# lhoyer/improving_segmentation_with_selfsupervised_depth

Measured on AMD Instinct MI355X. Metric: train images/sec, ResNet-101 joint seg+depth @512x1024, higher is better.
Workload: dtype f32

## Files before the change

### improving_segmentation_with_selfsupervised_depth_amd/csrc/conv_igemm.hip

```cpp
#include <type_traits>
#include "segsde_common.h"
#include "conv_small.h"
#include "winograd.h"
#include <cstdlib>
#include <mutex>
#include <cstring>

namespace {

struct ConvP {
  const float* x0; const float* x1; const float* w; const float* bias;
  float* y; float* y2;
  int B, H, W, C0, C1, ld0, ld1, up0;
  int Ho, Wo, N, ldy, ldy2, nsplit;
  int KH, KW, stride, dil, pad, pad_mode, in_div;
  int Ctot, Ktot, M, act, sum2x2;
  int vecout;
  int nb, ne;
  const float* zero;
  int kh0, khs, kw0, kws, KWf, Kfull, os, oph, opw, OHf, OWf;
  double* stats;
  int accum;
  const float* agy; int agld, agkind;
  unsigned mg1, mg2; int sf1, sf2, d1, d2;
  unsigned mgC, mgKW; int sfC, sfKW;
  int lin;
  int padw, wtap, osfast;
  int submap;
  int tapskip;
  long wbstride;
  int cmp;
};
constexpr int SEGSDE_PAD_CLAMP_ = 3;

struct KInfo {
  const float* src; int ld, Hs, Ws, shift, dh, dw, cc; bool valid;
};

__device__ __forceinline__ int fast_div(int n, unsigned magic, int shift) {
  return magic ? (int)(__umulhi((unsigned)n, magic) >> shift) : n;
}

__device__ __forceinline__ KInfo decode_k(const ConvP& p, int k) {
  KInfo t;
  t.valid = k < p.Ktot;
  const int kk = t.valid ? k : 0;
  const int tap = fast_div(kk, p.mgC, p.sfC), c = kk - tap * p.Ctot;
  const int kh = fast_div(tap, p.mgKW, p.sfKW), kw = tap - kh * p.KW;
  t.dh = kh * p.dil - p.pad;
  t.dw = kw * p.dil - p.pad;
  if (c < p.C0) { t.src = p.x0; t.ld = p.ld0; t.cc = c; t.shift = p.up0; }
  else { t.src = p.x1; t.ld = p.ld1; t.cc = c - p.C0; t.shift = 0; }
  t.Hs = p.H >> t.shift;
  t.Ws = p.W >> t.shift;
  return t;
}
// ... 678 lines not shown
      if (sn < pe.ne) {
        double* pr = pe.stats + ((long)(mt * R + sl) * 2) * pe.N + sn;
        pr[0] = ((s8[0] + s8[1]) + (s8[2] + s8[3])) + ((s8[4] + s8[5]) + (s8[6] + s8[7]));
        pr[pe.N] = ((q8[0] + q8[1]) + (q8[2] + q8[3])) + ((q8[4] + q8[5]) + (q8[6] + q8[7]));
      }
    }
    constexpr int CQ = BN / 4, RPP = 256 / CQ;
    const int cq = tid % CQ, rr = tid / CQ;
    const int n = n0 + 4 * cq;
    {
      const int nend = n0 + BN < pe.ne ? n0 + BN : pe.ne;
      const bool side1 = n0 >= pe.nsplit;
      if ((!pe.submap || pe.osfast) && m0 + BM <= pe.M && (side1 || nend <= pe.nsplit)) {
        constexpr int NR = BM / RPP;
        const long row0 = pe.submap ? out_row(pe, m0) : (long)m0;
        float* dbase = side1 ? pe.y2 + (row0 * pe.ldy2 + (n0 - pe.nsplit)) : pe.y + (row0 * pe.ldy + n0);
        const unsigned ld = (unsigned)(side1 ? pe.ldy2 : pe.ldy) * (unsigned)pe.os;
        const segsde_rsrc rd = segsde_make_rsrc(dbase);
        const unsigned vo = n < pe.ne ? ((unsigned)rr * ld + 4u * cq) * 4u : SEGSDE_OOB;
        const unsigned step = (unsigned)RPP * ld * 4u;
        const bool ag = pe.agy && !side1;
        const unsigned agl = (unsigned)pe.agld * (unsigned)pe.os;
        const segsde_rsrc ra = segsde_make_rsrc(ag ? pe.agy + (row0 * pe.agld + n0) : pe.zero);
        const unsigned voa = (ag && n < pe.ne) ? ((unsigned)rr * agl + 4u * cq) * 4u : SEGSDE_OOB;
        const unsigned stepa = (unsigned)RPP * agl * 4u;
        const float* cp = Ct + rr * BN + 4 * cq;
        float4 o[NR];
        if (pe.accum) {
          unsigned so = 0;
#pragma unroll
          for (int t = 0; t < NR; ++t) { o[t] = segsde_buffer_load4(rd, vo, so); so += step; }
        }
        unsigned so = 0, soa = 0;
        if (pe.accum && pe.act != SEGSDE_ACT_NONE) {
#pragma unroll
          for (int t = 0; t < NR; ++t) {
            float4 v = *reinterpret_cast<const float4*>(cp + t * RPP * BN);
            v.x += o[t].x; v.y += o[t].y; v.z += o[t].z; v.w += o[t].w;
            if (pe.act == SEGSDE_ACT_ELU) {
              v.x = v.x > 0.f ? v.x : __expf(fminf(v.x, 0.f)) - 1.f; v.y = v.y > 0.f ? v.y : __expf(fminf(v.y, 0.f)) - 1.f;
              v.z = v.z > 0.f ? v.z : __expf(fminf(v.z, 0.f)) - 1.f; v.w = v.w > 0.f ? v.w : __expf(fminf(v.w, 0.f)) - 1.f;
            } else {
              v.x = segsde_act(v.x, pe.act); v.y = segsde_act(v.y, pe.act); v.z = segsde_act(v.z, pe.act); v.w = segsde_act(v.w, pe.act);
            }
            segsde_buffer_store4(rd, vo, so, v);
            so += step;
          }
          return;
        }
#pragma unroll
        for (int t = 0; t < NR; ++t) {
          float4 v = *reinterpret_cast<const float4*>(cp + t * RPP * BN);
          if (ag) {
            const float4 yv = segsde_buffer_load4(ra, voa, soa);
            v.x *= segsde_act_grad_from_out(yv.x, pe.agkind); v.y *= segsde_act_grad_from_out(yv.y, pe.agkind);
            v.z *= segsde_act_grad_from_out(yv.z, pe.agkind); v.w *= segsde_act_grad_from_out(yv.w, pe.agkind);
          }
          if (pe.accum) { v.x += o[t].x; v.y += o[t].y; v.z += o[t].z; v.w += o[t].w; }
          segsde_buffer_store4(rd, vo, so, v);
          so += step; soa += stepa;
        }
        return;
      }
    }
    if (n < pe.ne) {
      float* dst; long ld; int nn;
      if (n < pe.nsplit) { dst = pe.y; ld = pe.ldy; nn = n; }
      else { dst = pe.y2; ld = pe.ldy2; nn = n - pe.nsplit; }
      if (pe.accum) {
        constexpr int NR = BM / RPP;
        float4 o[NR];
        const float* ag = (pe.agy && n < pe.nsplit) ? pe.agy + nn : nullptr;
#pragma unroll
        for (int t = 0; t < NR; ++t) {
          const int m = m0 + rr + t * RPP;
          o[t] = make_float4(0.f, 0.f, 0.f, 0.f);
          if (m < pe.M) o[t] = *reinterpret_cast<const float4*>(dst + out_row(pe, m) * ld + nn);
        }
#pragma unroll
        for (int t = 0; t < NR; ++t) {
          const int ml = rr + t * RPP, m = m0 + ml;
          if (m < pe.M) {
            float4 v = *reinterpret_cast<const float4*>(Ct + ml * BN + 4 * cq);
            if (ag) {
              const float4 yv = *reinterpret_cast<const float4*>(ag + out_row(pe, m) * pe.agld);
              v.x *= segsde_act_grad_from_out(yv.x, pe.agkind); v.y *= segsde_act_grad_from_out(yv.y, pe.agkind);
              v.z *= segsde_act_grad_from_out(yv.z, pe.agkind); v.w *= segsde_act_grad_from_out(yv.w, pe.agkind);
            }
            v.x += o[t].x; v.y += o[t].y; v.z += o[t].z; v.w += o[t].w;
            if (pe.act == SEGSDE_ACT_ELU) {
              v.x = v.x > 0.f ? v.x : __expf(fminf(v.x, 0.f)) - 1.f; v.y = v.y > 0.f ? v.y : __expf(fminf(v.y, 0.f)) - 1.f;
              v.z = v.z > 0.f ? v.z : __expf(fminf(v.z, 0.f)) - 1.f; v.w = v.w > 0.f ? v.w : __expf(fminf(v.w, 0.f)) - 1.f;
            } else if (pe.act != SEGSDE_ACT_NONE) {
              v.x = segsde_act(v.x, pe.act); v.y = segsde_act(v.y, pe.act); v.z = segsde_act(v.z, pe.act); v.w = segsde_act(v.w, pe.act);
            }
            *reinterpret_cast<float4*>(dst + out_row(pe, m) * ld + nn) = v;
          }
        }
      } else if (pe.agy && n < pe.nsplit) {
        const float* ag = pe.agy + nn;
#pragma unroll 4
        for (int ml = rr; ml < BM; ml += RPP) {
          const int m = m0 + ml;
          if (m < pe.M) {
            const long row = out_row(pe, m);
            float4 v = *reinterpret_cast<const float4*>(Ct + ml * BN + 4 * cq);
            const float4 yv = *reinterpret_cast<const float4*>(ag + row * pe.agld);
            v.x *= segsde_act_grad_from_out(yv.x, pe.agkind); v.y *= segsde_act_grad_from_out(yv.y, pe.agkind);
            v.z *= segsde_act_grad_from_out(yv.z, pe.agkind); v.w *= segsde_act_grad_from_out(yv.w, pe.agkind);
            *reinterpret_cast<float4*>(dst + row * ld + nn) = v;
          }
        }
      } else {
#pragma unroll 4
        for (int ml = rr; ml < BM; ml += RPP) {
          const int m = m0 + ml;
          if (m < pe.M) {
            float4* q = reinterpret_cast<float4*>(dst + out_row(pe, m) * ld + nn);
            *q = *reinterpret_cast<const float4*>(Ct + ml * BN + 4 * cq);
          }
        }
      }
// ... 634 lines not shown
  const unsigned long long num = 1ULL << (31 + l);
  magic = (unsigned)((num + (unsigned long long)d - 1) / (unsigned long long)d);
  shift = l - 1;
}
void set_divs(ConvP& p) {
  p.d1 = p.sum2x2 ? (p.Ho >> 1) * (p.Wo >> 1) : p.Ho * p.Wo;
  p.d2 = p.sum2x2 ? (p.Wo >> 1) : p.Wo;
  magic_for(p.d1, p.mg1, p.sf1);
  magic_for(p.d2, p.mg2, p.sf2);
  magic_for(p.Ctot, p.mgC, p.sfC);
  magic_for(p.KW, p.mgKW, p.sfKW);
}

ConvP make_params(const segsde_conv_desc* d, const float* x0, const float* x1, const float* w, const float* bias,
                  float* y, float* y2) {
  ConvP p;
  p.x0 = x0; p.x1 = x1 ? x1 : x0; p.w = w; p.bias = bias; p.y = y; p.y2 = y2 ? y2 : y;
  p.B = d->B; p.H = d->H; p.W = d->W; p.C0 = d->C0; p.C1 = d->C1; p.ld0 = d->ld0; p.ld1 = d->C1 ? d->ld1 : d->ld0;
  p.up0 = d->up0; p.Ho = d->Ho; p.Wo = d->Wo; p.N = d->Cout; p.ldy = d->ldy;
  p.ldy2 = d->ldy2 ? d->ldy2 : d->ldy; p.nsplit = y2 ? d->nsplit : d->Cout;
  p.KH = d->KH; p.KW = d->KW; p.stride = d->stride; p.dil = d->dil; p.pad = d->pad; p.pad_mode = d->pad_mode;
  p.in_div = d->in_div < 1 ? 1 : d->in_div;
  p.Ctot = d->C0 + d->C1; p.Ktot = d->KH * d->KW * p.Ctot; p.M = d->B * d->Ho * d->Wo; p.act = d->act;
  p.sum2x2 = d->sum2x2;
  set_divs(p);
  p.nb = 0; p.ne = p.N;
  p.vecout = (p.N % 4 == 0) && (p.ldy % 4 == 0) && (p.ldy2 % 4 == 0) && (p.nsplit % 4 == 0) && aligned16(p.y) &&
             aligned16(p.y2);
  p.zero = zero_page();
  p.kh0 = 0; p.khs = 1; p.kw0 = 0; p.kws = 1; p.KWf = p.KW; p.Kfull = p.Ktot; p.os = 1; p.oph = 0; p.opw = 0; p.OHf = p.Ho; p.OWf = p.Wo;
  p.stats = nullptr;
  p.accum = d->accumulate ? 1 : 0;
  p.cmp = (d->compute == 1 || d->compute == 2) ? d->compute : 0;
  p.agy = nullptr; p.agld = 0; p.agkind = 0;
  p.lin = d->KH == 1 && d->KW == 1 && d->stride == 1 && d->pad == 0 && d->in_div <= 1 && !d->up0 && !d->sum2x2 && d->C1 == 0 &&
          d->H == d->Ho && d->W == d->Wo;
  p.padw = p.pad; p.wtap = p.Ctot; p.osfast = 0; p.submap = 0;
  p.tapskip = (d->pad_mode == SEGSDE_PAD_ZERO && d->dil > 1 && d->KH > 1 && d->in_div <= 1 && !d->up0 && !d->sum2x2 &&
               d->stride == 1) ? 1 : 0;
  p.wbstride = 0;
  return p;
}


bool vec_ok(const ConvP& p) {
  return (p.Ctot % 4 == 0) && (p.C0 % 4 == 0) && (p.ld0 % 4 == 0) && (p.ld1 % 4 == 0) && aligned16(p.x0) &&
         aligned16(p.x1) && aligned16(p.w);
}

int validate(const segsde_conv_desc* d) {
  if (!d || d->B <= 0 || d->H <= 0 || d->W <= 0 || d->C0 <= 0 || d->C1 < 0 || d->Cout <= 0) return SEGSDE_ERR_SHAPE;
  if (d->KH <= 0 || d->KW <= 0 || d->stride <= 0 || d->dil <= 0 || d->pad < 0) return SEGSDE_ERR_SHAPE;
  if (d->up0 && ((d->H & 1) || (d->W & 1))) return SEGSDE_ERR_SHAPE;
  if (d->pad_mode == SEGSDE_PAD_REFLECT && (d->pad >= d->H || d->pad >= d->W)) return SEGSDE_ERR_SHAPE;
  if (d->pad_mode == SEGSDE_PAD_REFLECT_ADJOINT &&
      (d->KH != 3 || d->KW != 3 || d->stride != 1 || d->dil != 1 || d->pad != 1 || d->in_div > 1 || d->C1 != 0 ||
       d->H != d->Ho || d->W != d->Wo || d->H < 2 || d->W < 2))
    return SEGSDE_ERR_SHAPE;
  if (d->ld0 < d->C0 || (d->C1 && d->ld1 < d->C1) || d->ldy <= 0) return SEGSDE_ERR_SHAPE;
  if (d->compute == 3) return SEGSDE_ERR_UNSUPPORTED;
  return 0;
}

bool fast_ok(const ConvP& p) {
  const long e0 = (long)p.B * (p.H >> p.up0) * (p.W >> p.up0) * p.ld0;
  const long e1 = (long)p.B * p.H * p.W * p.ld1;
  return vec_ok(p) && (p.Ctot % 32 == 0) && (p.C1 == 0 || p.C0 % 32 == 0) && p.in_div <= 2 && e0 < (1L << 31) &&
// ... 175 lines not shown
}

extern "C" int segsde_reflect_adjoint_borders(const segsde_conv_desc* d, const float* dy, const float* wdpack, float* y,
                                              const float* act_out, int act_ld, int act_kind, void* stream) {
  if (!dy || !wdpack || !y) return SEGSDE_ERR_NULL;
  ConvP p;
  if (int e = borders_params(d, dy, wdpack, y, act_out, act_ld, act_kind, p)) return e;
  return launch_adjoint_by_borders(p, static_cast<hipStream_t>(stream), false);
}

extern "C" long segsde_conv2d_stats_rows(const segsde_conv_desc* d) {
  if (validate(d)) return 0;
  float dummy[4];
  const ConvP p = make_params(d, dummy, dummy, dummy, nullptr, reinterpret_cast<float*>(16), nullptr);
  return stats_rows(d, p);
}

extern "C" int segsde_conv2d_forward(const segsde_conv_desc* d, const float* x0, const float* x1, const float* wpack,
                                     const float* bias, float* y, float* y2, void* stream) {
  return segsde_conv2d_forward_stats(d, x0, x1, wpack, bias, y, y2, nullptr, stream);
}

extern "C" int segsde_conv2d_forward_stats(const segsde_conv_desc* d, const float* x0, const float* x1, const float* wpack,
                                           const float* bias, float* y, float* y2, double* stats, void* stream) {
  return segsde_conv2d_dgrad_actgrad(d, x0, x1, wpack, bias, y, y2, stats, nullptr, 0, 0, stream);
}

extern "C" int segsde_conv2d_dgrad_actgrad(const segsde_conv_desc* d, const float* x0, const float* x1, const float* wpack,
                                           const float* bias, float* y, float* y2, double* stats, const float* act_out,
                                           int act_ld, int act_kind, void* stream) {
  if (int e = validate(d)) return e;
  if (!x0 || !wpack || !y || (d->C1 && !x1)) return SEGSDE_ERR_NULL;
  ConvP p = make_params(d, x0, x1, wpack, bias, y, y2);
  if (act_out) {
    if (stats || bias || d->act != 0 || act_kind < SEGSDE_ACT_RELU || act_kind > SEGSDE_ACT_SIGMOID || act_ld < p.nsplit ||
        (act_ld % 4) || !aligned16(act_out) || d->in_div > 1)
      return SEGSDE_ERR_UNSUPPORTED;
    p.agy = act_out; p.agld = act_ld; p.agkind = act_kind;
  }
  if (stats) {
    if (stats_rows(d, p) == 0) return SEGSDE_ERR_UNSUPPORTED;
    p.stats = stats;
  }
  const bool parity_split = d->in_div == 2 && d->stride == 1 && (d->dil & 1) && d->pad_mode == SEGSDE_PAD_ZERO && !d->sum2x2 &&
                            d->C1 == 0 && !d->up0 && !bias && d->act == 0 && !y2 && p.vecout;
  if (d->accumulate) {
    if (y2 || bias || d->act != 0 || d->sum2x2 || (d->in_div > 1 && !parity_split) || !p.vecout || d->Cout == 1 || d->C0 % 4 != 0 ||
        d->C0 == 1 || (d->pad_mode == SEGSDE_PAD_REFLECT_ADJOINT && !igemm_fast_ok(p)))
      return SEGSDE_ERR_UNSUPPORTED;
  }
  hipStream_t s = static_cast<hipStream_t>(stream);
  const bool plain3x3 = d->KH == 3 && d->KW == 3 && d->stride == 1 && d->dil == 1 && d->pad == 1 && d->C1 == 0 && !d->up0 &&
                        d->in_div <= 1 && !d->sum2x2 && d->H == d->Ho && d->W == d->Wo;
  if (plain3x3 && d->Cout == 1 && d->pad_mode != SEGSDE_PAD_REFLECT_ADJOINT && segsde_c1_supported(d->C0, d->ld0) &&
      aligned16(x0) && aligned16(wpack))
    return probing() ? 0 : segsde_c1_forward(x0, d->ld0, d->B, d->H, d->W, d->C0, wpack, bias, d->pad_mode == SEGSDE_PAD_REFLECT, d->act, y,
                             d->ldy, stream);
  if (plain3x3 && d->C0 == 1 && d->pad_mode != SEGSDE_PAD_REFLECT && !bias && d->act == 0 &&
      segsde_c1_supported(d->Cout, p.ldy) && p.vecout)
    return probing() ? 0 : segsde_c1_dgrad(x0, d->ld0, d->B, d->H, d->W, d->Cout, wpack, d->pad_mode == SEGSDE_PAD_REFLECT_ADJOINT, y, p.ldy,
                           y2, p.ldy2, p.nsplit, p.agy, p.agld, p.agkind, stream);
  const bool plain1x1 = d->KH == 1 && d->KW == 1 && d->stride == 1 && d->pad == 0 && d->C1 == 0 && !d->up0 && d->in_div <= 1 &&
                        !d->sum2x2 && d->H == d->Ho && d->W == d->Wo;
  if (plain1x1 && !stats && !p.agy && d->C0 % 4 != 0 && d->ld0 == d->C0 && aligned16(x0) && !bias && d->act == 0 && !y2 &&
      segsde_skinny_supported(d->C0, d->Cout) && p.vecout)
    return probing() ? 0 : segsde_skinny_nk(x0, d->C0, wpack, (long)d->B * d->H * d->W, d->Cout, y, p.ldy, stream);
  if (parity_split) {
    bool ok = true;
    ConvP sub[4]; int nsub = 0; bool empty = false;
    for (int ph = 0; ph < 2 && ok; ++ph)
      for (int pw = 0; pw < 2 && ok; ++pw) {
// ... 836 lines not shown
```

### improving_segmentation_with_selfsupervised_depth_amd/functional.py

```python
import collections
import weakref

import torch
from torch.autograd import Function as _TorchFunction

from . import hipops as H


class Function(_TorchFunction):

    @classmethod
    def apply(cls, *args):
        return super(_TorchFunction, cls).apply(*args)


FUSIONS = {}


def _grad_dest(param):
    from . import ddp
    return ddp.grad_destination(param) if ddp._GRAD_DEST else None


def fp32_region(fn):
# ... 95 lines not shown

def to_nchw_dense(x_nhwc):
    return _ToNCHWDense.apply(x_nhwc)


class StemFn(Function):

    @staticmethod
    def forward(ctx, image, weight, mean, std, stats_out=None, wstem=None):
        xpad = H.stem_input(image, mean, std)
        if wstem is None:
            wstem = H.stem_pack(weight)
        C = weight.shape[1]
        if stats_out is not None:
            y, part = H.stem_forward(xpad, wstem, C, want_stats=True)
            stats_out.append(part)
        else:
            y = H.stem_forward(xpad, wstem, C)
        ctx.C = C
        ctx.save_for_backward(xpad)
        return y

    @staticmethod
    def backward(ctx, dy):
        (xpad,) = ctx.saved_tensors
        dw = H.stem_wgrad(xpad, _c(dy), ctx.C) if ctx.needs_input_grad[1] else None
        return None, dw, None, None, None, None


class ConvFn(Function):

    @staticmethod
    def forward(ctx, x0, x1, weight, bias, g, act, stats_out=None, grad_box=None, packs=None, x0_act=None, act_box=None,
                fold_cache=None, wino_cache=None, skip_box=None):
        ctx.grad_box = grad_box
        ctx.skip_box = skip_box
        ctx.x0_act, ctx.act_box = x0_act, act_box
        x0 = _c(x0) if x0.stride(-1) != 1 else x0
        ctx.wd = None
        ctx.wd_gen = None
        if packs is not None:
            wp, ctx.wd = packs
            ctx.wd_gen = getattr(ctx.wd, "_segsde_gen", None)
        elif ctx.needs_input_grad[0] or (x1 is not None and ctx.needs_input_grad[1]):
            wp, ctx.wd = H.pack_weight_both(weight)
        else:
            wp = H.pack_weight(weight, False)
        ctx.wp = wp if g.reflect else None
        ctx.fold = None
        ctx.wino = None
        up_f = 2 if g.up0 else 1
        kn = H.winograd_fused_ok(g, x0.shape[0], x0.shape[1] * up_f, x0.shape[2] * up_f)
        kn_d2 = (x1 is not None and g.up0 and (ctx.needs_input_grad[1])
                 and H.winograd_fused_dgrad2_ok(g, x0.shape[0], x0.shape[1] * up_f, x0.shape[2] * up_f))
        if kn or kn_d2 or (not g.up0 and H.winograd_ok(g, x0.shape[0], x0.shape[1], x0.shape[2])):
            knl = kn or kn_d2
            if (wino_cache is not None and wino_cache.get("key") is not None and wino_cache.get("key") == wino_cache.get("want")
                    and bool(wino_cache.get("kn")) == knl):
                ctx.wino = wino_cache["packs"]
            else:
                ctx.wino = H.winograd_pack(weight, kn=knl)
                if wino_cache is not None and wino_cache.get("want") is not None:
                    wino_cache["packs"], wino_cache["key"], wino_cache["kn"] = ctx.wino, wino_cache["want"], knl
        wino_f = None if (ctx.wino is None or (kn_d2 and not kn)) else ctx.wino[0]
        keep_v = wino_f is not None and not kn and ctx.needs_input_grad[2]
        H.WINO_V[0] = None
        if stats_out is not None:
            y, part = H.conv_forward(g, x0, x1, wp, bias, act, want_stats=True, wino=wino_f, keep_v=keep_v)
# ... 6 lines not shown
                    ctx.fold = H.upfold_pack(weight, g.C0)
                    if fold_cache is not None and fold_cache.get("want") is not None:
                        fold_cache["fold"], fold_cache["key"] = ctx.fold, fold_cache["want"]
            y = H.conv_forward(g, x0, x1, wp, bias, act, wfold=None if ctx.fold is None else ctx.fold[0], wino=wino_f, keep_v=keep_v)
        ctx.wino_v, H.WINO_V[0] = H.WINO_V[0], None
        ctx.g, ctx.act = g, act
        ctx.in_hw = (x0.shape[1] * (2 if g.up0 else 1), x0.shape[2] * (2 if g.up0 else 1))
        ctx.has_bias = bias is not None
        ctx.save_for_backward(x0, x1, weight)
        return y

    @staticmethod
    def backward(ctx, dy):
        x0, x1, weight = ctx.saved_tensors
        g = ctx.g
        dz = _c(dy)
        need_b = ctx.has_bias and ctx.needs_input_grad[3]
        dbias = None
        if need_b:
            stash = ctx.act_box.pop("dbias", None) if ctx.act_box is not None else None
            same = stash is not None and stash[0].data_ptr() == dz.data_ptr() and stash[0]._version == stash[1] == dz._version
            dbias = stash[2] if same else H.colsum(dz)
            fusion("bias_grad_from_activation_pass", bool(same))
        actgrad = (x0, ctx.x0_act) if ctx.x0_act is not None else None
        dx0 = dx1 = dw = None
        if ctx.needs_input_grad[0] or (x1 is not None and ctx.needs_input_grad[1]):
            wd = ctx.wd if ctx.wd is not None else H.pack_weight(weight, True)
            if ctx.wd_gen is not None and getattr(wd, "_segsde_gen", None) != ctx.wd_gen:
                raise RuntimeError("the weight packs of this graph were rebuilt by a later weight_pack_scope(model): a graph "
                                   "must be consumed before the next prepack of the same weights")
            dx0 = None
            box = ctx.grad_box
            if box is not None and box.get("g") is not None and x1 is None:
                dx0, dx1 = H.conv_dgrad(g, dz, wd, weight.detach(), ctx.in_hw, accumulate_into=box["g"], actgrad=actgrad,
                                        wino=None if ctx.wino is None else ctx.wino[1], wfpack=ctx.wp)
                if dx0 is not None:
                    box["fused"] = True
            if dx0 is None:
                sbox = ctx.skip_box if (x1 is not None and ctx.needs_input_grad[1]) else None
                dx0, dx1 = H.conv_dgrad(g, dz, wd, weight.detach(), ctx.in_hw, actgrad=actgrad, fold=ctx.fold,
                                        need0=ctx.needs_input_grad[0], need1=x1 is not None and ctx.needs_input_grad[1],
                                        wino=None if ctx.wino is None else ctx.wino[1],
                                        accumulate_skip_into=None if sbox is None else sbox.get("g"), wfpack=ctx.wp)
                if sbox is not None and dx1 is not None:
                    if H.SKIP_ACCUMULATED[0]:
                        sbox["fused"] = True
                    elif sbox.get("publish") and sbox.get("g") is None and dx1.is_contiguous():
                        sbox["g"] = dx1
                        sbox["fused"] = True
                if box is not None and box.get("publish") and box.get("g") is None and x1 is None and not g.up0 \
                        and dx0.is_contiguous():
                    box["g"] = dx0
                    box["fused"] = True
            if actgrad is not None and ctx.needs_input_grad[0]:
                fusion("activation_backward_in_dgrad_epilogue", bool(H.ACTGRAD_FUSED[0]))
            if not ctx.needs_input_grad[0]:
                dx0 = None
            if x1 is None or not ctx.needs_input_grad[1]:
                dx1 = None
        if ctx.needs_input_grad[2]:
            dw = H.conv_wgrad(g, x0, x1, dz, wino_v=ctx.wino_v, out=_grad_dest(weight))
            ctx.wino_v = None
        return dx0, dx1, dw, dbias, None, None, None, None, None, None, None, None, None, None


class ActGradFn(Function):

    passes = 0

    @staticmethod
    def forward(ctx, y, act, box):
        ctx.act, ctx.box = act, box
        ctx.save_for_backward(y)
        return y.view_as(y)

    @staticmethod
    def backward(ctx, dy):
        (y,) = ctx.saved_tensors
        ActGradFn.passes += 1
        fusion("activation_backward_in_dgrad_epilogue", False)
        dz, dbias = H.act_backward(_c(dy), y, ctx.act, need_dbias=bool(ctx.box.get("need_dbias")))
        if dbias is not None:
            ctx.box["dbias"] = (dz, dz._version, dbias)
        return dz, None, None


class BNActFn(Function):

    @staticmethod
    def forward(ctx, x, gamma, beta, residual, running_mean, running_var, training, momentum, eps, act, drop_p, seed,
                partials=None, grad_box=None, nbt=None):
        ctx.grad_box = grad_box
        x = _c(x)
        if training and partials is not None:
            mean, invstd = H.bn_stats_from_partials(partials, x.numel() // x.shape[-1], running_mean, running_var, momentum,
                                                    eps, update_running=running_mean is not None, num_batches_tracked=nbt)
        elif training:
            mean, invstd = H.bn_stats(x, running_mean, running_var, momentum, eps, update_running=running_mean is not None,
                                      num_batches_tracked=nbt)
        else:
            mean, invstd = H.bn_eval_stats(running_mean, running_var, eps)
        y = H.bn_apply(x, mean, invstd, gamma, beta, residual, act, drop_p, seed)
        remask = act in ("none", "relu") and residual is None and not drop_p
        ctx.cfg = (act, drop_p, seed, training, residual is not None, remask)
        ctx.beta_param = beta
        ctx.save_for_backward(x, gamma, beta if remask else None, mean, invstd, None if remask else y)
        return y

    @staticmethod
    def backward(ctx, dy):
        x, gamma, beta, mean, invstd, y = ctx.saved_tensors
        act, drop_p, seed, training, has_res, remask = ctx.cfg
        want_g = gamma is not None and ctx.needs_input_grad[1]
        bp = ctx.beta_param
        dx, dres, dgamma, dbeta = H.bn_backward(_c(dy), y, x, mean, invstd, gamma, act, drop_p, seed, batch_stats=training,
                                                need_dx=ctx.needs_input_grad[0],
                                                need_dres=has_res and ctx.needs_input_grad[3], beta=beta,
                                                dgamma_out=_grad_dest(gamma) if want_g else None,
                                                dbeta_out=_grad_dest(bp) if (want_g and bp is not None and ctx.needs_input_grad[2]) else None)
        ctx.beta_param = None
        if gamma is None or not ctx.needs_input_grad[1]:
            dgamma = dbeta = None
        if ctx.grad_box is not None and dres is not None:
            ctx.grad_box["g"] = dres
        return dx, dgamma, dbeta, dres, None, None, None, None, None, None, None, None, None, None, None


class SplitFn(Function):

    fused_count = 0

    @staticmethod
    def forward(ctx, x, box):
        ctx.box = box
        return x.view_as(x), x.view_as(x)

    @staticmethod
    def backward(ctx, g_main, g_skip):
        box = ctx.box
        fused = bool(box.get("fused")) and g_main is not None and g_skip is not None and g_main.data_ptr() == g_skip.data_ptr()
        box.clear()
        if fused:
            SplitFn.fused_count += 1
            fusion("residual_grad_accumulate", True)
            return g_main, None
        if g_main is None:
            return g_skip, None
        if g_skip is None:
            return g_main, None
        fusion("residual_grad_accumulate", False)
        return g_main + g_skip, None


class FanoutFn(Function):

    shared_count = 0

    @staticmethod
# ... 414 lines not shown
```

### improving_segmentation_with_selfsupervised_depth_amd/hipops.py

```python
import ctypes
import os
import threading

import torch

from . import _lib
from ._lib import ConvDesc, check

ACT = {"none": 0, "relu": 1, "elu": 2, "sigmoid": 3}


class _Slot(threading.local):

    def __init__(self, default=None):
        self.default = default
        self.v = default

    def __getattr__(self, name):
        if name == "v":
            return self.__dict__.setdefault("v", self.__dict__.get("default"))
        raise AttributeError(name)

    def __getitem__(self, i):
        return self.v
# ... 538 lines not shown
        WINO_V[0] = None
        r = _winograd("conv_fwd", g, x0, x1, wino, g.Cout, want_stats, flops, _tag(g, H, W), bias=bias, act=act, reflect=g.reflect,
                      keep_v=keep_v and WINOGRAD_KEEP_V)
        if r is not None:
            return r if want_stats else r[0]
    if wfold is not None and not want_stats:
        rc = _timed("conv_fwd", flops, x0, lambda: _lib.lib().segsde_conv2d_forward_upfold(
            ctypes.byref(d), _p(_f32(x0)), _p(x1), _p(wpack), _p(wfold), _p(bias), _p(y), _stream(x0)), _tag(g, H, W) + " fold",
            executed=flops * _fold_frac(g))
        if rc == 0:
            UPFOLD_TAKEN["fwd"] += 1
            _note_compute(d, 4, "fwd")
            return y
        if rc != -4:
            check(rc, "conv2d_forward_upfold")
    part = None
    if want_stats and bias is None and act == "none":
        rows = int(_lib.lib().segsde_conv2d_stats_rows(ctypes.byref(d)))
        if rows > 0:
            part = torch.empty((rows, 2, g.Cout), dtype=torch.float64, device=x0.device)
    _timed("conv_fwd", flops, x0, lambda: check(_lib.lib().segsde_conv2d_forward_stats(
        ctypes.byref(d), _p(_f32(x0)), _p(x1), _p(wpack), _p(bias), _p(y), None, _p(part), _stream(x0)), "conv2d_forward"),
        _tag(g, H, W), executed=flops_x)
    _note_compute(d, 0, "fwd")
    return (y, part) if want_stats else y


ACTGRAD_FUSED = _Slot(False)


SKIP_ACCUMULATED = _Slot(False)


def conv_dgrad(g, dy, wdpack, w_oihw, in_hw, need0=True, need1=True, accumulate_into=None, actgrad=None, fold=None, wino=None,
               accumulate_skip_into=None, wfpack=None):
    B, Ho, Wo, Cout = dy.shape
    H, W = in_hw
    assert Cout == g.Cout
    ACTGRAD_FUSED[0] = False
    SKIP_ACCUMULATED[0] = False
    dx1 = torch.empty((B, H, W, g.C1), dtype=torch.float32, device=dy.device) if g.C1 else None
    L = _lib.lib()
    flops = 2.0 * B * Ho * Wo * Cout * g.CinAlg * g.k * g.k
    ag_y, ag_ld, ag_kind = None, 0, 0
    if actgrad is not None:
        ag_y, ag_kind = actgrad[0], ACT[actgrad[1]]
        ag_ld = nhwc_ld(ag_y)

    if isinstance(wino, _KnPack):
        ext = actgrad is not None or g.reflect
        if (winograd_fused_ok(g, B, H, W, dgrad=True) and (Ho, Wo) == (H, W) and (not ext or WINO_FUSED_DGRAD_EXT)
                and (not g.reflect or B * H * W >= WINO_FUSED_REFLECT_DGRAD_MIN_PIX)
                and (not g.reflect or (wfpack is not None and BORDERS2 and H >= 4 and W >= 4 and g.C0 % 32 == 0 and Cout % 32 == 0 and Cout <= 1024)
                     or reflect_borders_ok(B, H, W, Cout, g.C0, nhwc_ld(dy), ag_ld))
                and (actgrad is None or (ag_ld % 4 == 0 and ag_y.data_ptr() % 16 == 0))):
            r = winograd_fused("conv_dgrad", dy, wino, tag=_tag(g, H, W), accumulate_into=accumulate_into, actgrad=actgrad,
                               adjoint=(g, wdpack, wfpack) if g.reflect else None)
            if r is not None:
                ACTGRAD_FUSED[0] = actgrad is not None
                return r[0], None
    elif (wino is not None and accumulate_into is None and actgrad is None and not g.reflect and g.C1 == 0
            and winograd_ok(g, B, H, W, dgrad=True) and (Ho, Wo) == (H, W)):
        r = _winograd("conv_dgrad", g, dy, None, wino, g.C0, False, flops, _tag(g, H, W))
        if r is not None:
            return r[0], None

    def desc(sum2x2, accumulate=0):
        return ConvDesc(B=B, H=Ho, W=Wo, C0=Cout, C1=0, ld0=nhwc_ld(dy), ld1=0, up0=0, Ho=H, Wo=W, Cout=g.Cin, ldy=g.C0,
                        ldy2=g.C1, nsplit=g.C0, KH=g.k, KW=g.k, stride=1, dil=g.dil, pad=(g.k - 1) * g.dil - g.pad,
                        pad_mode=PAD_REFLECT_ADJOINT if g.reflect else PAD_ZERO, in_div=g.stride, act=0, sum2x2=sum2x2,
                        accumulate=accumulate, compute=g.compute)

    def launch(d, y, y2, fuse):
        return L.segsde_conv2d_dgrad_actgrad(ctypes.byref(d), _p(_f32(dy)), None, _p(wdpack), None, _p(y), _p(y2), None,
                                             _p(ag_y) if fuse else None, ag_ld if fuse else 0, ag_kind if fuse else 0,
                                             _stream(dy))

    def finish_unfused(dx0):
        if actgrad is None or dx0 is None:
            return dx0
# ... 918 lines not shown
```

### improving_segmentation_with_selfsupervised_depth_amd/models/layers.py

```python
import os

import torch
from torch import nn

from .. import functional as Fn
from .. import hipops as H
from ..hipops import ConvGeom


def _seed():
    return int(torch.randint(0, 2 ** 31 - 1, (1,)).item())


_NO_FUSED_STATS = bool(int(os.environ.get("SEGSDE_NO_FUSED_STATS", "0")))


GRAPH_SAFE_DROPOUT = [False]
_PACK_SCOPE = [0, 0]


class weight_pack_scope:

    def __init__(self, model=None):
        self._model = model
# ... 50 lines not shown
        assert self.kernel_size[0] == self.kernel_size[1] and self.stride[0] == self.stride[1]

    def _weight_packs(self, weight):
        d = self.__dict__
        if not _PACK_SCOPE[0]:
            d["_packs"] = None
            return None
        key = (_PACK_SCOPE[0], weight._version, weight.data_ptr(), weight.device)
        if key != d["_pack_key"] or d["_packs"] is None:
            d["_packs"], d["_pack_key"] = H.pack_weight_both(weight), key
        return d["_packs"]

    def forward_image(self, image, mean, std):
        if not H.stem_ok(image, self) or (torch.is_grad_enabled() and image.requires_grad):
            return None
        wstem = None
        if _PACK_SCOPE[0]:
            key = (_PACK_SCOPE[0], self.weight._version, self.weight.data_ptr(), self.weight.device)
            if key != getattr(self, "_stem_key", None):
                self._stem_pack, self._stem_key = H.stem_pack(self.weight), key
            wstem = self._stem_pack
        if self.training and not _NO_FUSED_STATS and self._stats_wanted is not False:
            if self._stats_wanted is None and self._stats_offered:
                self._stats_wanted = False
                return Fn.StemFn.apply(image, self.weight, mean, std, None, wstem)
            if not self._stats_offered:
                self._stats_offered = True
            holder = []
            y = Fn.StemFn.apply(image, self.weight, mean, std, holder, wstem)
            y._bn_partials = (holder[0], y._version, self) if holder and holder[0] is not None else None
            return y
        return Fn.StemFn.apply(image, self.weight, mean, std, None, wstem)

    def forward(self, x, skip=None, up=False, act="none", grad_box=None, skip_box=None):
        c0 = x.shape[3]
        c1 = 0 if skip is None else skip.shape[3]
        weight = self.weight
        if skip is None and c0 > self.in_channels:
            weight = torch.nn.functional.pad(weight, (0, 0, 0, 0, 0, c0 - self.in_channels))
            packs = None
        else:
            assert c0 + c1 == self.in_channels, (c0, c1, self.in_channels)
            packs = self._weight_packs(weight)
        g = ConvGeom(c0, self.out_channels, self.kernel_size[0], self.stride[0], self.dilation[0], self.padding[0],
                     self.reflect, c1, up, cin_alg=self.in_channels if (skip is None and c0 > self.in_channels) else None)
        x0_act = None
        pre = getattr(x, "_preact", None)
        if pre is not None and pre[2] == x._version and torch.is_grad_enabled() and pre[0].requires_grad:
            x, x0_act = pre[0], pre[1]
        wc = self._wino_cache
        wc["want"] = (_PACK_SCOPE[0], weight._version, weight.data_ptr(), weight.device) if _PACK_SCOPE[0] else None
        if self.bias is None and act == "none" and self.training and not _NO_FUSED_STATS and self._stats_wanted is not False:
            if self._stats_wanted is None and self._stats_offered:
                self._stats_wanted = False
                return Fn.ConvFn.apply(x, skip, weight, self.bias, g, act, None, grad_box, packs, x0_act, None, None, wc)
            if not self._stats_offered:
                self._stats_offered = True
            holder = []
            y = Fn.ConvFn.apply(x, skip, weight, self.bias, g, act, holder, grad_box, packs, x0_act, None, None, wc)
            y._bn_partials = (holder[0], y._version, self) if holder and holder[0] is not None else None
            return y
        if act == "none":
            return Fn.ConvFn.apply(x, skip, weight, self.bias, g, act, None, grad_box, packs, x0_act, None, None, wc)
        box = {"need_dbias": self.bias is not None and self.bias.requires_grad}
        fc = self._fold_cache
        fc["want"] = (_PACK_SCOPE[0], weight._version, weight.data_ptr(), weight.device, c0) if (_PACK_SCOPE[0] and up) else None
        yz = Fn.ConvFn.apply(x, skip, weight, self.bias, g, act, None, grad_box, packs, x0_act, box, fc, wc, skip_box)
        if not (torch.is_grad_enabled() and yz.requires_grad):
            return yz
        y = Fn.ActGradFn.apply(yz, act, box)
        y._preact = (yz, act, y._version)
        return y


class BatchNorm2d(nn.BatchNorm2d):

    def forward(self, x, residual=None, act="none", drop_p=0.0, grad_box=None):
        training = self.training or (self.running_mean is None)
        nbt = self.num_batches_tracked if (self.training and self.track_running_stats
                                           and self.num_batches_tracked is not None) else None
        if self.momentum is None:
            momentum = 1.0 / float(int(self.num_batches_tracked) + 1) if nbt is not None else 0.0
        else:
            momentum = self.momentum
        if drop_p > 0 and GRAPH_SAFE_DROPOUT[0]:
            y = self.forward(x, residual, act, 0.0, grad_box)
            return torch.nn.functional.dropout(y, drop_p, True)
        seed = _seed() if drop_p > 0 else 0
        partials = getattr(x, "_bn_partials", None) if training else None
        if partials is not None:
            partials, version, producer = partials
            if partials.shape[-1] != self.num_features or x._version != version:
                partials = None
            elif producer._stats_wanted is not True:
                producer._stats_wanted = True
        if training:
            Fn.fusion("bn_stats_from_conv_epilogue", partials is not None)
        return Fn.BNActFn.apply(x, self.weight, self.bias, residual, self.running_mean, self.running_var, training,
                                momentum, self.eps, act, drop_p, seed, partials, grad_box, nbt)
```

### improving_segmentation_with_selfsupervised_depth_amd/models/resnet_encoder.py

```python
import errno
import os

import numpy as np
import torch
from torch import nn

from .. import functional as Fn
from .layers import Conv2d, BatchNorm2d


class BasicBlock(nn.Module):
    expansion = 1

    def __init__(self, inplanes, planes, stride=1, downsample=None, dilation=1):
        super().__init__()
        if dilation > 1:
            raise NotImplementedError("Dilation > 1 not supported in BasicBlock")
        self.conv1 = Conv2d(inplanes, planes, 3, stride, 1, bias=False)
        self.bn1 = BatchNorm2d(planes)
        self.relu = nn.ReLU(inplace=True)
        self.conv2 = Conv2d(planes, planes, 3, 1, 1, bias=False)
        self.bn2 = BatchNorm2d(planes)
        self.downsample = downsample

    def forward(self, x, x_ds=None, box=None):
        if self.downsample is None and x.requires_grad:
            box = {}
            xm, xs = Fn.SplitFn.apply(x, box)
            o = self.bn1(self.conv1(xm, grad_box=box), act="relu")
            return self.bn2(self.conv2(o), residual=xs, act="relu", grad_box=box)
        if self.downsample is not None and x_ds is None and x.requires_grad:
            (x, x_ds), box = Fn.fan_feature(x, 0, 2)
        idt = x if self.downsample is None else self.downsample[1](self.downsample[0](x if x_ds is None else x_ds, grad_box=box))
        o = self.bn1(self.conv1(x, grad_box=box), act="relu")
        return self.bn2(self.conv2(o), residual=idt, act="relu")


class Bottleneck(nn.Module):
    expansion = 4

    def __init__(self, inplanes, planes, stride=1, downsample=None, dilation=1):
        super().__init__()
        self.conv1 = Conv2d(inplanes, planes, 1, bias=False)
        self.bn1 = BatchNorm2d(planes)
        self.conv2 = Conv2d(planes, planes, 3, stride, dilation, dilation, bias=False)
        self.bn2 = BatchNorm2d(planes)
        self.conv3 = Conv2d(planes, planes * 4, 1, bias=False)
        self.bn3 = BatchNorm2d(planes * 4)
        self.relu = nn.ReLU(inplace=True)
        self.downsample = downsample

    def forward(self, x, x_ds=None, box=None):
        if self.downsample is None and x.requires_grad:
            box = {}
            xm, xs = Fn.SplitFn.apply(x, box)
            o = self.bn1(self.conv1(xm, grad_box=box), act="relu")
            o = self.bn2(self.conv2(o), act="relu")
            return self.bn3(self.conv3(o), residual=xs, act="relu", grad_box=box)
        if self.downsample is not None and x_ds is None and x.requires_grad:
            (x, x_ds), box = Fn.fan_feature(x, 0, 2)
        idt = x if self.downsample is None else self.downsample[1](self.downsample[0](x if x_ds is None else x_ds, grad_box=box))
        o = self.bn1(self.conv1(x, grad_box=box), act="relu")
        o = self.bn2(self.conv2(o), act="relu")
        return self.bn3(self.conv3(o), residual=idt, act="relu")


class ResNet(nn.Module):
    def __init__(self, block, layers, num_input_images=1, replace_stride_with_dilation=None):
        super().__init__()
        self.inplanes, self.dilation = 64, 1
        rswd = replace_stride_with_dilation or [False, False, False]
        self.conv1 = Conv2d(3 * num_input_images, 64, 7, 2, 3, bias=False)
        self.bn1 = BatchNorm2d(64)
        self.relu = nn.ReLU(inplace=True)
        self.maxpool = nn.MaxPool2d(3, 2, 1)
        self.layer1 = self._make_layer(block, 64, layers[0])
        self.layer2 = self._make_layer(block, 128, layers[1], stride=2, dilate=rswd[0])
        self.layer3 = self._make_layer(block, 256, layers[2], stride=2, dilate=rswd[1])
        self.layer4 = self._make_layer(block, 512, layers[3], stride=2, dilate=rswd[2])
        self.avgpool = nn.Identity()
        self.fc = nn.Identity()
        for m in self.modules():
            if isinstance(m, nn.Conv2d):
                nn.init.kaiming_normal_(m.weight, mode="fan_out", nonlinearity="relu")
            elif isinstance(m, nn.BatchNorm2d):
                nn.init.constant_(m.weight, 1)
                nn.init.constant_(m.bias, 0)

    def _make_layer(self, block, planes, blocks, stride=1, dilate=False):
# ... 97 lines not shown
```

### include/segsde_hip.h

```cpp
#ifndef SEGSDE_HIP_H
#define SEGSDE_HIP_H
#include <stddef.h>
#include <stdint.h>

#ifdef __cplusplus
extern "C" {
#endif

#define SEGSDE_ABI_VERSION 15

enum { SEGSDE_ERR_NULL = -1, SEGSDE_ERR_SHAPE = -2, SEGSDE_ERR_WORKSPACE = -3, SEGSDE_ERR_UNSUPPORTED = -4 };
enum { SEGSDE_ACT_NONE = 0, SEGSDE_ACT_RELU = 1, SEGSDE_ACT_ELU = 2, SEGSDE_ACT_SIGMOID = 3 };
enum { SEGSDE_DTYPE_F32 = 0, SEGSDE_DTYPE_I64 = 1, SEGSDE_DTYPE_U8 = 2 };
enum { SEGSDE_PAD_ZERO = 0, SEGSDE_PAD_REFLECT = 1, SEGSDE_PAD_REFLECT_ADJOINT = 2 };

int segsde_abi_version(void);

typedef struct segsde_conv_desc {
  int B, H, W;
  int C0, C1;
  int ld0, ld1;
  int up0;
  int Ho, Wo, Cout;
  int ldy, ldy2, nsplit;
  int KH, KW, stride, dil, pad;
  int pad_mode;
  int in_div;
  int act;
  int sum2x2;
  int accumulate;
  int compute;
} segsde_conv_desc;

enum { SEGSDE_DIR_FORWARD = 0, SEGSDE_DIR_DGRAD = 1, SEGSDE_DIR_WGRAD = 2, SEGSDE_DIR_UPFOLD = 4 };
int segsde_conv_compute_taken(const segsde_conv_desc* d, int direction);
int segsde_split_bf16_planes(const float* x, long n, unsigned short* h, unsigned short* m, unsigned short* l, void* stream);

int segsde_conv2d_forward(const segsde_conv_desc* d, const float* x0, const float* x1, const float* wpack,
                          const float* bias, float* y, float* y2, void* stream);
long segsde_conv2d_stats_rows(const segsde_conv_desc* d);
int segsde_conv2d_forward_stats(const segsde_conv_desc* d, const float* x0, const float* x1, const float* wpack,
                                const float* bias, float* y, float* y2, double* stats, void* stream);
int segsde_conv2d_dgrad_actgrad(const segsde_conv_desc* d, const float* x0, const float* x1, const float* wpack,
                                const float* bias, float* y, float* y2, double* stats, const float* act_out, int act_ld,
                                int act_kind, void* stream);

size_t segsde_conv2d_wgrad_workspace(const segsde_conv_desc* d);
int segsde_conv2d_wgrad(const segsde_conv_desc* d, const float* x0, const float* x1, const float* dy, int lddy,
                        float* dw_oihw, float* workspace, size_t workspace_bytes, void* stream);

int segsde_upfold_pack(const float* w_oihw, int Cout, int C0, int Ctot, float* wfold, float* wdfold, void* stream);
int segsde_conv2d_forward_upfold(const segsde_conv_desc* d, const float* x0, const float* x1, const float* wpack,
                                 const float* wfold, const float* bias, float* y, void* stream);
int segsde_conv2d_dgrad_upfold(const segsde_conv_desc* d, const float* dy, int lddy, const float* wdpack, const float* wfold,
                               const float* wdfold, float* dx0, float* dx1, int accumulate_dx1, const float* act_out, int act_ld,
                               int act_kind, void* stream);
size_t segsde_conv2d_wgrad_upfold_workspace(const segsde_conv_desc* d);
int segsde_conv2d_wgrad_upfold(const segsde_conv_desc* d, const float* x0, const float* x1, const float* dy, int lddy,
                               float* dw_oihw, float* workspace, size_t workspace_bytes, void* stream);

int segsde_stem_pack(const float* w_oihw, int Cout, int C, int cp, float* wstem, void* stream);
long segsde_stem7x7_stats_rows(int B, int Hp, int Wp, int cp, int Cout);
int segsde_stem7x7_forward(const float* xpad, int B, int Hp, int Wp, int cp, const float* wstem, int Cout, float* y, double* stats,
                           void* stream);
size_t segsde_stem7x7_wgrad_workspace(int B, int Hp, int Wp, int cp, int Cout);
int segsde_stem7x7_wgrad(const float* xpad, int B, int Hp, int Wp, int cp, const float* dy, int lddy, int Cout, int C,
                         float* dw_oihw, float* workspace, size_t workspace_bytes, void* stream);

int segsde_pack_weight(const float* w_oihw, float* out, int O, int I, int KH, int KW, int for_dgrad, void* stream);
int segsde_pack_weight_both(const float* w_oihw, float* out_fwd, float* out_dgrad, int O, int I, int KH, int KW,
                            void* stream);
typedef struct segsde_pack_job {
  const float* w; float* fwd; float* dgrad;
  int O, I, KH, KW, block0, reserved;
} segsde_pack_job;
// ... 194 lines not shown
```

Baseline: 63.58.

## Apply residual ReLU mask in conv1 dgrad epilogue after accumulation

```diff
diff --git a/improving_segmentation_with_selfsupervised_depth_amd/csrc/conv_igemm.hip b/improving_segmentation_with_selfsupervised_depth_amd/csrc/conv_igemm.hip
--- a/improving_segmentation_with_selfsupervised_depth_amd/csrc/conv_igemm.hip
+++ b/improving_segmentation_with_selfsupervised_depth_amd/csrc/conv_igemm.hip
@@ -22,6 +22,7 @@
   double* stats;
   int accum;
   const float* agy; int agld, agkind;
+  int agpost;
   unsigned mg1, mg2; int sf1, sf2, d1, d2;
   unsigned mgC, mgKW; int sfC, sfKW;
   int lin;
@@ -766,6 +767,21 @@
           for (int t = 0; t < NR; ++t) { o[t] = segsde_buffer_load4(rd, vo, so); so += step; }
         }
         unsigned so = 0, soa = 0;
+        if (pe.accum && pe.agpost) {
+          float4 yv[NR];
+#pragma unroll
+          for (int t = 0; t < NR; ++t) { yv[t] = segsde_buffer_load4(ra, voa, soa); soa += stepa; }
+#pragma unroll
+          for (int t = 0; t < NR; ++t) {
+            float4 v = *reinterpret_cast<const float4*>(cp + t * RPP * BN);
+            v.x += o[t].x; v.y += o[t].y; v.z += o[t].z; v.w += o[t].w;
+            v.x *= segsde_act_grad_from_out(yv[t].x, SEGSDE_ACT_RELU); v.y *= segsde_act_grad_from_out(yv[t].y, SEGSDE_ACT_RELU);
+            v.z *= segsde_act_grad_from_out(yv[t].z, SEGSDE_ACT_RELU); v.w *= segsde_act_grad_from_out(yv[t].w, SEGSDE_ACT_RELU);
+            segsde_buffer_store4(rd, vo, so, v);
+            so += step;
+          }
+          return;
+        }
         if (pe.accum && pe.act != SEGSDE_ACT_NONE) {
 #pragma unroll
           for (int t = 0; t < NR; ++t) {
@@ -816,12 +832,17 @@
           const int ml = rr + t * RPP, m = m0 + ml;
           if (m < pe.M) {
             float4 v = *reinterpret_cast<const float4*>(Ct + ml * BN + 4 * cq);
-            if (ag) {
+            if (ag && !pe.agpost) {
               const float4 yv = *reinterpret_cast<const float4*>(ag + out_row(pe, m) * pe.agld);
               v.x *= segsde_act_grad_from_out(yv.x, pe.agkind); v.y *= segsde_act_grad_from_out(yv.y, pe.agkind);
               v.z *= segsde_act_grad_from_out(yv.z, pe.agkind); v.w *= segsde_act_grad_from_out(yv.w, pe.agkind);
             }
             v.x += o[t].x; v.y += o[t].y; v.z += o[t].z; v.w += o[t].w;
+            if (ag && pe.agpost) {
+              const float4 yv = *reinterpret_cast<const float4*>(ag + out_row(pe, m) * pe.agld);
+              v.x *= segsde_act_grad_from_out(yv.x, pe.agkind); v.y *= segsde_act_grad_from_out(yv.y, pe.agkind);
+              v.z *= segsde_act_grad_from_out(yv.z, pe.agkind); v.w *= segsde_act_grad_from_out(yv.w, pe.agkind);
+            }
             if (pe.act == SEGSDE_ACT_ELU) {
               v.x = v.x > 0.f ? v.x : __expf(fminf(v.x, 0.f)) - 1.f; v.y = v.y > 0.f ? v.y : __expf(fminf(v.y, 0.f)) - 1.f;
               v.z = v.z > 0.f ? v.z : __expf(fminf(v.z, 0.f)) - 1.f; v.w = v.w > 0.f ? v.w : __expf(fminf(v.w, 0.f)) - 1.f;
@@ -1522,7 +1543,7 @@
   p.stats = nullptr;
   p.accum = d->accumulate ? 1 : 0;
   p.cmp = (d->compute == 1 || d->compute == 2) ? d->compute : 0;
-  p.agy = nullptr; p.agld = 0; p.agkind = 0;
+  p.agy = nullptr; p.agld = 0; p.agkind = 0; p.agpost = 0;
   p.lin = d->KH == 1 && d->KW == 1 && d->stride == 1 && d->pad == 0 && d->in_div <= 1 && !d->up0 && !d->sum2x2 && d->C1 == 0 &&
           d->H == d->Ho && d->W == d->Wo;
   p.padw = p.pad; p.wtap = p.Ctot; p.osfast = 0; p.submap = 0;
@@ -1764,11 +1785,14 @@
   if (int e = validate(d)) return e;
   if (!x0 || !wpack || !y || (d->C1 && !x1)) return SEGSDE_ERR_NULL;
   ConvP p = make_params(d, x0, x1, wpack, bias, y, y2);
+  const bool act_post = (act_kind & SEGSDE_ACTGRAD_AFTER_ACCUM) != 0;
+  act_kind &= ~SEGSDE_ACTGRAD_AFTER_ACCUM;
+  if (act_post && !(act_out && d->accumulate && act_kind == SEGSDE_ACT_RELU && p.lin)) return SEGSDE_ERR_UNSUPPORTED;
   if (act_out) {
     if (stats || bias || d->act != 0 || act_kind < SEGSDE_ACT_RELU || act_kind > SEGSDE_ACT_SIGMOID || act_ld < p.nsplit ||
         (act_ld % 4) || !aligned16(act_out) || d->in_div > 1)
       return SEGSDE_ERR_UNSUPPORTED;
-    p.agy = act_out; p.agld = act_ld; p.agkind = act_kind;
+    p.agy = act_out; p.agld = act_ld; p.agkind = act_kind; p.agpost = act_post ? 1 : 0;
   }
   if (stats) {
     if (stats_rows(d, p) == 0) return SEGSDE_ERR_UNSUPPORTED;
diff --git a/improving_segmentation_with_selfsupervised_depth_amd/functional.py b/improving_segmentation_with_selfsupervised_depth_amd/functional.py
--- a/improving_segmentation_with_selfsupervised_depth_amd/functional.py
+++ b/improving_segmentation_with_selfsupervised_depth_amd/functional.py
@@ -151,8 +151,9 @@
 
     @staticmethod
     def forward(ctx, x0, x1, weight, bias, g, act, stats_out=None, grad_box=None, packs=None, x0_act=None, act_box=None,
-                fold_cache=None, wino_cache=None, skip_box=None):
+                fold_cache=None, wino_cache=None, skip_box=None, mask_box=None):
         ctx.grad_box = grad_box
+        ctx.mask_box = mask_box
         ctx.skip_box = skip_box
         ctx.x0_act, ctx.act_box = x0_act, act_box
         x0 = _c(x0) if x0.stride(-1) != 1 else x0
@@ -225,8 +226,15 @@
             dx0 = None
             box = ctx.grad_box
             if box is not None and box.get("g") is not None and x1 is None:
-                dx0, dx1 = H.conv_dgrad(g, dz, wd, weight.detach(), ctx.in_hw, accumulate_into=box["g"], actgrad=actgrad,
-                                        wino=None if ctx.wino is None else ctx.wino[1], wfpack=ctx.wp)
+                mbox = ctx.mask_box
+                if mbox is not None and actgrad is None and ctx.needs_input_grad[0]:
+                    dx0, dx1 = H.conv_dgrad(g, dz, wd, weight.detach(), ctx.in_hw, accumulate_into=box["g"], actgrad=(x0, "relu"),
+                                            mask_sum=True, wino=None if ctx.wino is None else ctx.wino[1], wfpack=ctx.wp)
+                    if dx0 is not None:
+                        mbox["dz"] = (dx0, dx0._version)
+                if dx0 is None:
+                    dx0, dx1 = H.conv_dgrad(g, dz, wd, weight.detach(), ctx.in_hw, accumulate_into=box["g"], actgrad=actgrad,
+                                            wino=None if ctx.wino is None else ctx.wino[1], wfpack=ctx.wp)
                 if dx0 is not None:
                     box["fused"] = True
             if dx0 is None:
@@ -254,7 +262,7 @@
         if ctx.needs_input_grad[2]:
             dw = H.conv_wgrad(g, x0, x1, dz, wino_v=ctx.wino_v, out=_grad_dest(weight))
             ctx.wino_v = None
-        return dx0, dx1, dw, dbias, None, None, None, None, None, None, None, None, None, None
+        return dx0, dx1, dw, dbias, None, None, None, None, None, None, None, None, None, None, None
 
 
 class ActGradFn(Function):
@@ -282,8 +290,9 @@
 
     @staticmethod
     def forward(ctx, x, gamma, beta, residual, running_mean, running_var, training, momentum, eps, act, drop_p, seed,
-                partials=None, grad_box=None, nbt=None):
+                partials=None, grad_box=None, nbt=None, mask_box=None):
         ctx.grad_box = grad_box
+        ctx.mask_box = mask_box
         x = _c(x)
         if training and partials is not None:
             mean, invstd = H.bn_stats_from_partials(partials, x.numel() // x.shape[-1], running_mean, running_var, momentum,
@@ -297,7 +306,7 @@
         remask = act in ("none", "relu") and residual is None and not drop_p
         ctx.cfg = (act, drop_p, seed, training, residual is not None, remask)
         ctx.beta_param = beta
-        ctx.save_for_backward(x, gamma, beta if remask else None, mean, invstd, None if remask else y)
+        ctx.save_for_backward(x, gamma, beta if (remask or mask_box is not None) else None, mean, invstd, None if remask else y)
         return y
 
     @staticmethod
@@ -306,17 +315,30 @@
         act, drop_p, seed, training, has_res, remask = ctx.cfg
         want_g = gamma is not None and ctx.needs_input_grad[1]
         bp = ctx.beta_param
-        dx, dres, dgamma, dbeta = H.bn_backward(_c(dy), y, x, mean, invstd, gamma, act, drop_p, seed, batch_stats=training,
-                                                need_dx=ctx.needs_input_grad[0],
-                                                need_dres=has_res and ctx.needs_input_grad[3], beta=beta,
-                                                dgamma_out=_grad_dest(gamma) if want_g else None,
-                                                dbeta_out=_grad_dest(bp) if (want_g and bp is not None and ctx.needs_input_grad[2]) else None)
+        dgo = _grad_dest(gamma) if want_g else None
+        dbo = _grad_dest(bp) if (want_g and bp is not None and ctx.needs_input_grad[2]) else None
+        mbox, premasked = ctx.mask_box, False
+        if mbox is not None and mbox.get("claimed"):
+            st = mbox.pop("dz", None)
+            premasked = (st is not None and st[0].data_ptr() == dy.data_ptr() and st[0]._version == st[1] == dy._version
+                         and dy.shape == x.shape and dy.is_contiguous())
+            fusion("bn_residual_mask_in_dgrad_epilogue", premasked)
+        if premasked:
+            dx, _, dgamma, dbeta = H.bn_backward(dy, None, x, mean, invstd, gamma, "none", 0.0, 0, batch_stats=training,
+                                                 need_dx=ctx.needs_input_grad[0], need_dres=False, beta=beta,
+                                                 dgamma_out=dgo, dbeta_out=dbo)
+            dres = dy if ctx.needs_input_grad[3] else None
+        else:
+            dx, dres, dgamma, dbeta = H.bn_backward(_c(dy), y, x, mean, invstd, gamma, act, drop_p, seed, batch_stats=training,
+                                                    need_dx=ctx.needs_input_grad[0],
+                                                    need_dres=has_res and ctx.needs_input_grad[3], beta=beta if remask else None,
+                                                    dgamma_out=dgo, dbeta_out=dbo)
         ctx.beta_param = None
         if gamma is None or not ctx.needs_input_grad[1]:
             dgamma = dbeta = None
         if ctx.grad_box is not None and dres is not None:
             ctx.grad_box["g"] = dres
-        return dx, dgamma, dbeta, dres, None, None, None, None, None, None, None, None, None, None, None
+        return dx, dgamma, dbeta, dres, None, None, None, None, None, None, None, None, None, None, None, None
 
 
 class SplitFn(Function):
diff --git a/improving_segmentation_with_selfsupervised_depth_amd/hipops.py b/improving_segmentation_with_selfsupervised_depth_amd/hipops.py
--- a/improving_segmentation_with_selfsupervised_depth_amd/hipops.py
+++ b/improving_segmentation_with_selfsupervised_depth_amd/hipops.py
@@ -594,8 +594,11 @@
 SKIP_ACCUMULATED = _Slot(False)
 
 
+ACTGRAD_AFTER_ACCUM = 0x100
+
+
 def conv_dgrad(g, dy, wdpack, w_oihw, in_hw, need0=True, need1=True, accumulate_into=None, actgrad=None, fold=None, wino=None,
-               accumulate_skip_into=None, wfpack=None):
+               accumulate_skip_into=None, wfpack=None, mask_sum=False):
     B, Ho, Wo, Cout = dy.shape
     H, W = in_hw
     assert Cout == g.Cout
@@ -608,6 +611,10 @@
     if actgrad is not None:
         ag_y, ag_kind = actgrad[0], ACT[actgrad[1]]
         ag_ld = nhwc_ld(ag_y)
+    if mask_sum:
+        if accumulate_into is None or actgrad is None or actgrad[1] != "relu" or g.k != 1 or g.stride != 1 or isinstance(wino, _KnPack):
+            return None, None
+        ag_kind |= ACTGRAD_AFTER_ACCUM
 
     if isinstance(wino, _KnPack):
         ext = actgrad is not None or g.reflect
diff --git a/improving_segmentation_with_selfsupervised_depth_amd/models/layers.py b/improving_segmentation_with_selfsupervised_depth_amd/models/layers.py
--- a/improving_segmentation_with_selfsupervised_depth_amd/models/layers.py
+++ b/improving_segmentation_with_selfsupervised_depth_amd/models/layers.py
@@ -106,7 +106,7 @@
             return y
         return Fn.StemFn.apply(image, self.weight, mean, std, None, wstem)
 
-    def forward(self, x, skip=None, up=False, act="none", grad_box=None, skip_box=None):
+    def forward(self, x, skip=None, up=False, act="none", grad_box=None, skip_box=None, mask_box=None):
         c0 = x.shape[3]
         c1 = 0 if skip is None else skip.shape[3]
         weight = self.weight
@@ -127,15 +127,15 @@
         if self.bias is None and act == "none" and self.training and not _NO_FUSED_STATS and self._stats_wanted is not False:
             if self._stats_wanted is None and self._stats_offered:
                 self._stats_wanted = False
-                return Fn.ConvFn.apply(x, skip, weight, self.bias, g, act, None, grad_box, packs, x0_act, None, None, wc)
+                return Fn.ConvFn.apply(x, skip, weight, self.bias, g, act, None, grad_box, packs, x0_act, None, None, wc, None, mask_box)
             if not self._stats_offered:
                 self._stats_offered = True
             holder = []
-            y = Fn.ConvFn.apply(x, skip, weight, self.bias, g, act, holder, grad_box, packs, x0_act, None, None, wc)
+            y = Fn.ConvFn.apply(x, skip, weight, self.bias, g, act, holder, grad_box, packs, x0_act, None, None, wc, None, mask_box)
             y._bn_partials = (holder[0], y._version, self) if holder and holder[0] is not None else None
             return y
         if act == "none":
-            return Fn.ConvFn.apply(x, skip, weight, self.bias, g, act, None, grad_box, packs, x0_act, None, None, wc)
+            return Fn.ConvFn.apply(x, skip, weight, self.bias, g, act, None, grad_box, packs, x0_act, None, None, wc, None, mask_box)
         box = {"need_dbias": self.bias is not None and self.bias.requires_grad}
         fc = self._fold_cache
         fc["want"] = (_PACK_SCOPE[0], weight._version, weight.data_ptr(), weight.device, c0) if (_PACK_SCOPE[0] and up) else None
@@ -170,5 +170,9 @@
                 producer._stats_wanted = True
         if training:
             Fn.fusion("bn_stats_from_conv_epilogue", partials is not None)
-        return Fn.BNActFn.apply(x, self.weight, self.bias, residual, self.running_mean, self.running_var, training,
-                                momentum, self.eps, act, drop_p, seed, partials, grad_box, nbt)
+        mask_box = {} if (act == "relu" and residual is not None and not drop_p and torch.is_grad_enabled()) else None
+        y = Fn.BNActFn.apply(x, self.weight, self.bias, residual, self.running_mean, self.running_var, training,
+                             momentum, self.eps, act, drop_p, seed, partials, grad_box, nbt, mask_box)
+        if mask_box is not None and y.requires_grad:
+            y._bn_relu_box = (mask_box, y._version)
+        return y
diff --git a/improving_segmentation_with_selfsupervised_depth_amd/models/resnet_encoder.py b/improving_segmentation_with_selfsupervised_depth_amd/models/resnet_encoder.py
--- a/improving_segmentation_with_selfsupervised_depth_amd/models/resnet_encoder.py
+++ b/improving_segmentation_with_selfsupervised_depth_amd/models/resnet_encoder.py
@@ -53,8 +53,12 @@
     def forward(self, x, x_ds=None, box=None):
         if self.downsample is None and x.requires_grad:
             box = {}
+            prod = getattr(x, "_bn_relu_box", None)
+            mbox = prod[0] if (prod is not None and prod[1] == x._version and torch.is_grad_enabled()) else None
+            if mbox is not None:
+                mbox["claimed"] = True
             xm, xs = Fn.SplitFn.apply(x, box)
-            o = self.bn1(self.conv1(xm, grad_box=box), act="relu")
+            o = self.bn1(self.conv1(xm, grad_box=box, mask_box=mbox), act="relu")
             o = self.bn2(self.conv2(o), act="relu")
             return self.bn3(self.conv3(o), residual=xs, act="relu", grad_box=box)
         if self.downsample is not None and x_ds is None and x.requires_grad:
diff --git a/include/segsde_hip.h b/include/segsde_hip.h
--- a/include/segsde_hip.h
+++ b/include/segsde_hip.h
@@ -41,6 +41,7 @@
 long segsde_conv2d_stats_rows(const segsde_conv_desc* d);
 int segsde_conv2d_forward_stats(const segsde_conv_desc* d, const float* x0, const float* x1, const float* wpack,
                                 const float* bias, float* y, float* y2, double* stats, void* stream);
+#define SEGSDE_ACTGRAD_AFTER_ACCUM 0x100
 int segsde_conv2d_dgrad_actgrad(const segsde_conv_desc* d, const float* x0, const float* x1, const float* wpack,
                                 const float* bias, float* y, float* y2, double* stats, const float* act_out, int act_ld,
                                 int act_kind, void* stream);
```

Result: no change. 64.18, median of 6 (+0.9%).
